# itz-sayak/C-Users-Sayakdutta-Self-Supervised-Arbitrary-Scale-Point-Cloud-Upsampling-via-SNN

Measured on AMD Instinct MI355X. Metric: upsampled query-points/sec (kNN + fn fwd + rotate + fd fwd + displace), 4x scale, M=48 T=4, higher is better.
Workload: dtype f32 (GEMMs as 3 x f16 MFMA with f32 accumulation; outer kNN f64); 1 GPU; synthetic sphere N=5000 (seed 0), B=4096 grid queries per GPU per step, M=48, T=4, fn k=[24,18,12] emb 640, fd k=32 scales [8,16,32,48] emb 768, conditioned-random weights seed 0, in-patch kNN recomputed every batch; cloud_points=5000, neighbours=48, outer_knn=f64 brute force, parallelism=query shards x1

## Files before the change

c-users-sayakdutta-self-supervised-arbitrary-scale-point-cloud-upsampling-via-snn_amd/_lib.py:

```python
import ctypes
import os
from ctypes import POINTER, c_char_p, c_double, c_float, c_int, c_int32, c_int64, c_void_p

_HERE = os.path.dirname(os.path.abspath(__file__))
LIB_PATH = os.environ.get("SAPCU_LIB_PATH") or os.path.join(_HERE, "csrc", "libsapcu_hip.so")
EXACT_LIB_PATH = os.path.join(_HERE, "csrc", "libsapcu_hip_exact.so")

FN_TAPS = ("stem", "block1", "block2", "block3", "pooled", "enc", "logits")
FD_TAPS = ("fused0", "spikes", "knn", "pooled", "enc", "x0")
KIND_FN, KIND_FD = 0, 1
ABI_VERSION = 2


class SapcuLibraryError(RuntimeError):
    """The HIP library is absent or unloadable (never silently replaced by a CPU path)."""


class SapcuError(RuntimeError):
    """A C entry point returned a non-zero status: args = (code, text)."""


_SIGNATURES = {
    "sapcu_abi_version": (c_int, []),
    "sapcu_last_error": (c_char_p, []),
# ... 129 lines not shown
    "sapcu_plan_stats_f64": (c_int, [c_void_p, c_int64, c_void_p, c_int64, c_void_p, c_void_p, c_int, c_double, c_void_p, c_void_p,
                                     c_void_p, c_int64, c_void_p]),
}
SINKHORN_EXPORTS = tuple(_SINKHORN_SIGNATURES)

_RAY_SIGNATURES = {
    "sapcu_ray_mesh_workspace_bytes": (c_int64, [c_int64, c_int64, c_int64]),
    "sapcu_ray_mesh_f64": (c_int, [c_void_p, c_int64, c_void_p, c_int64, c_void_p, c_void_p, c_void_p, c_int64, c_double, c_void_p, c_void_p,
                                   c_void_p, c_void_p, c_int64, POINTER(c_int64), c_void_p]),
    "sapcu_ray_fd_samples_workspace_bytes": (c_int64, [c_int64, c_int64, c_int64]),
    "sapcu_ray_fd_samples_f64": (c_int, [c_void_p, c_int64, c_void_p, c_int64, c_void_p, c_void_p, c_void_p, c_void_p, c_int64, c_double] +
                                 [c_void_p] * 4 + [c_void_p, c_int64, POINTER(c_int64), c_void_p]),
}
RAY_EXPORTS = tuple(_RAY_SIGNATURES)

_NORMALS_SIGNATURES = {
    "sapcu_pca_normals_f64": (c_int, [c_void_p, c_int64, c_void_p, c_int64, c_int, POINTER(c_double), c_void_p, c_void_p, c_void_p, c_void_p]),
    "sapcu_normal_angles_f64": (c_int, [c_void_p, c_void_p, c_int64, c_int, c_double, c_void_p, c_void_p, c_void_p]),
}
NORMALS_EXPORTS = tuple(_NORMALS_SIGNATURES)

_INTERNAL_SIGNATURES = {
    "sapcu_internal_fold_affine_host": (c_int, [c_void_p, c_void_p, c_void_p, c_void_p, c_int, c_int, c_void_p, c_void_p]),
    "sapcu_internal_point_mesh_tuned": (c_int, [c_void_p, c_int64, c_void_p, c_int64, c_void_p, c_int64, c_double, c_double, c_int, c_int, c_void_p,
                                                c_void_p, c_void_p, c_void_p, c_int64, POINTER(c_int64), c_void_p]),
    "sapcu_internal_sinkhorn_split": (c_int, [c_int64, c_int64, POINTER(c_int64)]),
    "sapcu_internal_softmin_split_f64": (c_int, [c_void_p, c_int64, c_void_p, c_int64, c_void_p, c_int, c_double, c_int, c_void_p, c_void_p,
                                                 c_int64, c_void_p]),
    "sapcu_internal_ray_mesh_tuned": (c_int, [c_void_p, c_int64, c_void_p, c_int64, c_void_p, c_void_p, c_void_p, c_int64, c_double, c_double,
                                              c_int, c_double, c_int, c_void_p, c_void_p, c_void_p, c_void_p, c_int64, POINTER(c_int64),
                                              c_void_p]),
}
_lib = None


def load(path=None):
    global _lib
    if _lib is not None and path is None:
        return _lib
    p = path or LIB_PATH
    if not os.path.exists(p):
        raise SapcuLibraryError(
            "HIP library not built: %s is missing. Run `make -C %s` (needs hipcc, gfx950). "
            "There is no CPU fallback." % (p, os.path.dirname(p)))
    try:
        lib = ctypes.CDLL(p)
# ... 34 lines not shown
```

c-users-sayakdutta-self-supervised-arbitrary-scale-point-cloud-upsampling-via-snn_amd/csrc/model.hip:

```cpp
#include <stdarg.h>
#include <stdlib.h>

#include <new>
#include <vector>

#include "common.h"
#include "ops.h"

namespace sapcu {

static thread_local char g_err[512] = "";

void set_error(const char* fmt, ...) {
    va_list ap;
    va_start(ap, fmt);
    vsnprintf(g_err, sizeof(g_err), fmt, ap);
    va_end(ap);
}

enum FnSlot {
    FN_STEM_W = 0, FN_STEM_B, FN_STEM_LIF,
    FN_BLK0 = 3,
    FN_FINAL_W = FN_BLK0 + 63, FN_FINAL_B, FN_FINAL_LIF,
    FN_FCOUT_W, FN_FCOUT_B,
    FN_MLP0_W, FN_MLP0_B, FN_MLP1_W, FN_MLP1_B, FN_MLP2_W, FN_MLP2_B,
    FN_HEAD_W, FN_HEAD_B, FN_LN_W, FN_LN_B,
// ... 35 lines not shown
struct sapcu_model {
    int kind = 0;
    int kv[3] = {0, 0, 0};
    int k = 0, nscale = 0;
    int ks[8] = {0, 0, 0, 0, 0, 0, 0, 0};
    int32_t* ks_dev = nullptr;
    int* gate_dev = nullptr;
    bool sf16 = true;
    void* w16_hi = nullptr;
    void* w16_lo = nullptr;
    void* chain_w = nullptr;
    int* ovf_dev = nullptr;
    int emb = 0, T = 0, heads = 0;
    int64_t chunk = 0;
    int64_t ws_budget = 0;
    bool opt_bt = true;
    bool opt_chain = true;
    bool opt_chain_wide = false;
    bool opt_chain_fill = true;
    bool opt_chain_trim = true;
    bool opt_shortk = true;
    bool opt_fn_maxfuse = true;
    bool opt_fn_fold_out = true;
    bool opt_fd_maxfuse = true;
    bool opt_fd_split = true;
    bool opt_fd_fused = true;
    bool opt_fd_x0 = true;
    void* fde_w = nullptr;
    int64_t fde_off[5] = {0, 0, 0, 0, 0};
    float* fde_nprm = nullptr;
    float* blob = nullptr;
    int64_t blob_floats = 0;
    int64_t fold_w[3] = {0, 0, 0}, fold_b[3] = {0, 0, 0};
    std::vector<int64_t> dir;
    const float* p(int slot) const { return blob + dir[slot]; }
};

namespace sapcu {

static inline int64_t imax(int64_t a, int64_t b) { return a > b ? a : b; }
static inline int imin(int a, int b) { return a < b ? a : b; }

static bool split_rows_gemm_on_big_tile(const GemmArgs& g, bool allow_bt) { return allow_bt && gemm_sf16_bt_ok(g); }

int launch_gemm_split_rows(const GemmArgs& g, hipStream_t st, bool allow_bt) {
    if (split_rows_gemm_on_big_tile(g, allow_bt)) return launch_gemm_sf16_bt(g, st);
    return launch_gemm_sf16_ring(g, st);
}

static void fold_affine_f64(const float* w1, const float* b1, const float* w2, const float* b2, int d, int n, float* w_fold,
                            float* b_fold) {
    std::vector<double> acc((size_t)d);
    for (int i = 0; i < n; ++i) {
        for (int k = 0; k < d; ++k) acc[k] = 0.0;
        double bs = 0.0;
        for (int j = 0; j < d; ++j) {
            const double a = (double)w2[(int64_t)i * d + j];
            const float* row = w1 + (int64_t)j * d;
            for (int k = 0; k < d; ++k) acc[k] += a * (double)row[k];
            bs += a * (double)b1[j];
        }
        for (int k = 0; k < d; ++k) w_fold[(int64_t)i * d + k] = (float)acc[k];
        b_fold[i] = (float)(bs + (double)b2[i]);
    }
}

static bool env_is(const char* name, const char* value) {
    const char* e = getenv(name);
    return e && strcmp(e, value) == 0;
}

static void read_env_switches(sapcu_model* m) {
    m->sf16 = !env_is("SAPCU_GEMM", "f32");
    m->opt_bt = !env_is("SAPCU_BT", "0");
    m->opt_chain = !env_is("SAPCU_CHAIN", "0");
    m->opt_chain_wide = env_is("SAPCU_CHAIN", "wide");
    m->opt_chain_fill = !env_is("SAPCU_CHAIN_FILL", "0");
    m->opt_chain_trim = !env_is("SAPCU_CHAIN_TRIM", "0");
    m->opt_shortk = !env_is("SAPCU_SHORTK", "0");
    m->opt_fn_maxfuse = !env_is("SAPCU_FN_MAXFUSE", "0");
    m->opt_fn_fold_out = !env_is("SAPCU_FN_FOLD_OUT", "0");
    m->opt_fd_maxfuse = !env_is("SAPCU_FD_MAXFUSE", "0");
    m->opt_fd_split = !env_is("SAPCU_FD_SPLIT", "0");
    m->opt_fd_fused = !env_is("SAPCU_FD_FUSED", "0");
    m->opt_fd_x0 = !env_is("SAPCU_FD_X0", "0");
    const char* ce = getenv("SAPCU_CHUNK");
    m->chunk = ce ? atoll(ce) : 0;
    if (m->chunk < 0) m->chunk = 0;
    const char* be = getenv("SAPCU_WS_BUDGET_MB");
    m->ws_budget = (be ? atoll(be) : 20480) * (int64_t)(1 << 20);
    if (m->ws_budget < (int64_t)(64 << 20)) m->ws_budget = (int64_t)(64 << 20);
}

static void free_model(sapcu_model* m) {
    void* const owned[] = {m->w16_hi, m->w16_lo, m->chain_w, m->ovf_dev, m->blob, m->ks_dev, m->gate_dev, m->fde_w, m->fde_nprm};
    for (void* p : owned)
        if (p) (void)hipFree(p);
    delete m;
}

static int run_gemm(const sapcu_model* m, GemmArgs& g, hipStream_t st) {
    const bool have16 = m && m->sf16 && g.w >= m->blob && g.w < m->blob + m->blob_floats;
    if (have16) {
        const int64_t off = g.w - m->blob;
        g.w16_hi = (const _Float16*)m->w16_hi + off;
        g.w16_lo = (const _Float16*)m->w16_lo + off;
        g.ovf = m->ovf_dev;
        if (g.a_split) return launch_gemm_split_rows(g, st, m->opt_bt);
        if (m->opt_shortk && gemm_shortk_ok(g)) return launch_gemm_shortk(g, st);
        if (g.max_out) {
            set_error("run_gemm: a direct max output needs the short-K kernel");
            return SAPCU_ERR_ARG;
        }
        if (g.k % 64 == 0) return launch_gemm_sf16(g, st);
    }
    if (g.a_split || g.c_split || g.c2_split) {
        set_error("run_gemm: split-row operands need the split-f16 kernels");
        return SAPCU_ERR_ARG;
// ... 237 lines not shown
                SAPCU_CHECK_HIP(hipMemcpy2DAsync((char*)taps[SAPCU_FN_TAP_BLOCK1 + l] + s * mp * 64 * 4, 64 * 4,
                                                 out, 192 * 4, 64 * 4, (size_t)P, hipMemcpyDeviceToDevice, st));
            }
            fin = out;
            ldin = 192;
        }
        if (m->sf16 && m->opt_fn_maxfuse) {
            GemmArgs g;
            memset(&g, 0, sizeof(g));
            g.a = W.cat; g.r = P; g.k = 192; g.lda = 192; g.w = m->p(FN_FINAL_W); g.n = m->emb; g.bias = m->p(FN_FINAL_B);
            g.ldc = m->emb; g.epi = EPI_LIF_MAX; g.lif = m->p(FN_FINAL_LIF); g.lif_T = m->T;
            g.max_keys = reinterpret_cast<unsigned*>(W.B1); g.max_m = mp;
            const bool direct = m->opt_shortk && mp == 48;
            if (direct) g.max_out = W.pooled;
            else SAPCU_CHECK_HIP(hipMemsetAsync(g.max_keys, 0, (size_t)cb * m->emb * 4, st));
            SAPCU_TRY(run_gemm(m, g, st));
            if (!direct) SAPCU_TRY(launch_decode_max_keys(g.max_keys, cb * m->emb, W.pooled, st));
        } else {
            SAPCU_TRY(gemm(m, W.cat, P, 192, 192, m->p(FN_FINAL_W), m->emb, m->p(FN_FINAL_B), W.B1, m->emb, EPI_LIF, st,
                           m->p(FN_FINAL_LIF), m->T));
            SAPCU_TRY(launch_rowgroup_max(W.B1, cb, mp, m->emb, W.pooled, st));
        }
        SAPCU_TRY(tap_copy(taps, SAPCU_FN_TAP_POOLED, s * m->emb * 4, W.pooled, cb * m->emb * 4, st));
        SAPCU_TRY(gemm(m, W.pooled, cb, m->emb, m->emb, m->p(FN_FCOUT_W), 2048, m->p(FN_FCOUT_B), W.enc, 2048, EPI_BIAS, st));
        SAPCU_TRY(tap_copy(taps, SAPCU_FN_TAP_ENC, s * 2048 * 4, W.enc, cb * 2048 * 4, st));
        SAPCU_TRY(gemm(m, W.enc, cb, 2048, 2048, m->p(FN_MLP0_W), 1024, m->p(FN_MLP0_B), W.h1, 1024, EPI_GELU, st));
        SAPCU_TRY(gemm(m, W.h1, cb, 1024, 1024, m->p(FN_MLP1_W), 512, m->p(FN_MLP1_B), W.h2, 512, EPI_GELU, st));
        SAPCU_TRY(gemm(m, W.h2, cb, 512, 512, m->p(FN_MLP2_W), 256, m->p(FN_MLP2_B), W.h3, 256, EPI_GELU, st));
        SAPCU_TRY(launch_fn_tail(W.h3, cb, 256, m->p(FN_HEAD_W), m->p(FN_HEAD_B), m->p(FN_LN_W), m->p(FN_LN_B), W.logits,
                                 normals + s * 3, st));
        SAPCU_TRY(tap_copy(taps, SAPCU_FN_TAP_LOGITS, s * 3 * 4, W.logits, cb * 3 * 4, st));
    }
    return SAPCU_OK;
}

struct FdPlan {
    int64_t cb;
    int kmax0, kk;
    bool fused;
    bool x0path;
    bool maxfuse;
    int64_t agg_rows(int mp) const { return maxfuse ? 1 : mp; }
};

static bool fd_encoder_fused(const sapcu_model* m, int mp) {
    return m->sf16 && m->opt_fd_fused && m->fde_w && m->fde_nprm && fd_encoder_ok(mp, m->nscale, m->emb, m->T);
}

static bool fd_x0_path(const sapcu_model* m, int mp) {
// ... 173 lines not shown
    ma.pooled = W.POOLED; ma.tap_spikes = c.tap(SAPCU_FD_TAP_SPIKES); ma.gate = m->gate_dev;
    return launch_fd_msc(ma, st);
}

static int fd_msc_from_slabs(const sapcu_model* m, const FdPlan& pl, const FdWs& W, const FdChunk& c, bool split_spikes, hipStream_t st) {
    const int T = m->T, emb = m->emb;
    const int64_t P = c.P();
    if (c.tap(SAPCU_FD_TAP_SPIKES)) {
        for (int t = 0; t < T; ++t)
            SAPCU_CHECK_HIP(hipMemcpyAsync(c.tap(SAPCU_FD_TAP_SPIKES) + ((int64_t)t * c.b + c.s) * c.mp * 960,
                                           W.SPK + (int64_t)t * P * 960, P * 960 * 4, hipMemcpyDeviceToDevice, st));
    }
    if (pl.maxfuse) {
        GemmArgs mg = fd_msc_gemm_args(m, W, c);
        SAPCU_CHECK_HIP(hipMemsetAsync(mg.max_keys, 0, (size_t)T * c.cb * emb * 4, st));
        mg.a_split = split_spikes ? 1 : 0;
        SAPCU_TRY(run_gemm(m, mg, st));
        return launch_decode_max_keys(mg.max_keys, (int64_t)T * c.cb * emb, W.POOLED, st);
    }
    SAPCU_TRY(gemm(m, W.SPK, (int64_t)T * P, 960, 960, m->p(FD_MSC_W), emb, m->p(FD_MSC_B), W.AGG, emb, EPI_LRELU, st));
    return launch_rowgroup_max(W.AGG, (int64_t)T * c.cb, c.mp, emb, W.POOLED, st);
}

static int fd_temporal_decoder(const sapcu_model* m, const FdWs& W, const FdChunk& c, float* dist, hipStream_t st) {
    const int T = m->T, emb = m->emb;
    const int64_t cb = c.cb, s = c.s;
    if (c.tap(SAPCU_FD_TAP_POOLED)) {
        for (int t = 0; t < T; ++t)
            SAPCU_CHECK_HIP(hipMemcpyAsync(c.tap(SAPCU_FD_TAP_POOLED) + ((int64_t)t * c.b + s) * emb, W.POOLED + (int64_t)t * cb * emb,
                                           cb * emb * 4, hipMemcpyDeviceToDevice, st));
    }
    SAPCU_TRY(launch_fd_temporal(W.POOLED, T, cb, emb, m->p(FD_TI_W), m->p(FD_SNNFC), W.ENC, st));
    SAPCU_TRY(tap_copy(c.taps, SAPCU_FD_TAP_ENC, s * emb * 4, W.ENC, cb * emb * 4, st));
    SAPCU_TRY(gemm(m, W.ENC, cb, emb, emb, m->p(FD_FCIN_W), 256, m->p(FD_FCIN_B), W.D1, 256, EPI_GELU, st));
    SAPCU_TRY(gemm(m, W.D1, cb, 256, 256, m->p(FD_R0_FC0_W), 128, m->p(FD_R0_FC0_B), W.D2a, 128, EPI_GELU, st));
    SAPCU_TRY(gemm(m, W.D1, cb, 256, 256, m->p(FD_R0_PROJ_W), 128, m->p(FD_R0_PROJ_B), W.D2b, 128, EPI_BIAS, st));
    SAPCU_TRY(gemm(m, W.D2a, cb, 128, 128, m->p(FD_R0_FC4_W), 128, m->p(FD_R0_FC4_B), W.D2c, 128, EPI_RESID_GELU, st, nullptr, 0, W.D2b,
                   128));
    SAPCU_TRY(gemm(m, W.D2c, cb, 128, 128, m->p(FD_R1_FC0_W), 64, m->p(FD_R1_FC0_B), W.D3a, 64, EPI_GELU, st));
    SAPCU_TRY(gemm(m, W.D2c, cb, 128, 128, m->p(FD_R1_PROJ_W), 64, m->p(FD_R1_PROJ_B), W.D3b, 64, EPI_BIAS, st));
    SAPCU_TRY(gemm(m, W.D3a, cb, 64, 64, m->p(FD_R1_FC4_W), 64, m->p(FD_R1_FC4_B), W.D3c, 64, EPI_RESID_GELU, st, nullptr, 0, W.D3b, 64));
    SAPCU_TRY(gemm(m, W.D3c, cb, 64, 64, m->p(FD_QKV_W), 192, m->p(FD_QKV_B), W.QKV, 192, EPI_BIAS, st));
    return launch_fd_tail(W.D3c, W.QKV, cb, m->heads, m->p(FD_WO_T), m->p(FD_BO), m->p(FD_LN_W), m->p(FD_LN_B), m->p(FD_WH_T),
                          m->p(FD_BH), m->p(FD_WD), m->p(FD_BD), W.ATT, dist + s, st);
}

static int fd_forward(const sapcu_model* m, const float* patch, int64_t b, int mp, const int32_t* knn_force,
                      float* dist, void* ws, int64_t ws_bytes, void* const* taps, hipStream_t st) {
    const FdPlan pl = fd_plan(m, b, mp);
    const FdWs W = fd_ws_layout(ws_align256(ws), m, pl, mp);
    if (ws_bytes < (int64_t)W.bytes + 256) {
        set_error("fd_forward: workspace %lld B < required %lld B", (long long)ws_bytes, (long long)W.bytes + 256);
        return SAPCU_ERR_WORKSPACE;
// ... 296 lines not shown
            if (m->dir[i] < 0 || m->dir[i] >= blob_floats || (m->dir[i] & 3)) {
                set_error("model_create: slot %d offset %lld out of range / unaligned", i, (long long)m->dir[i]);
                rc = SAPCU_ERR_ARG;
                break;
            }
    }
    auto hip_ok = [&](hipError_t e, const char* what) {
        if (e != hipSuccess && rc == SAPCU_OK) {
            set_error("model_create: %s failed: %s", what, hipGetErrorString(e));
            rc = SAPCU_ERR_HIP;
        }
    };
    if (rc == SAPCU_OK) {
        int64_t total = blob_floats;
        if (kind == SAPCU_KIND_FN && m->opt_fn_fold_out) {
            total = (total + 63) & ~(int64_t)63;
            for (int l = 0; l < 3; ++l) {
                m->fold_w[l] = total;
                total += (int64_t)64 * (128 << l);
                m->fold_b[l] = total;
                total += 64;
            }
        }
        m->blob_floats = total;
        hip_ok(hipMalloc((void**)&m->blob, (size_t)total * 4), "hipMalloc(blob)");
        if (rc == SAPCU_OK) hip_ok(hipMemcpy(m->blob, blob, (size_t)blob_floats * 4, hipMemcpyDeviceToDevice), "copy blob");
        if (rc == SAPCU_OK && total > blob_floats)
            hip_ok(hipMemset(m->blob + blob_floats, 0, (size_t)(total - blob_floats) * 4), "memset folded parameters");
        for (int l = 0; l < 3 && rc == SAPCU_OK && total > blob_floats; ++l) {
            const int d = 128 << l, sb = FN_BLK0 + l * B_SLOTS;
            const int64_t need[4] = {(int64_t)d * d, d, (int64_t)64 * d, 64};
            static const int slot[4] = {B_OUT_W, B_OUT_B, B_FC2_W, B_FC2_B};
            std::vector<float> h[4], wf((size_t)64 * d), bf(64);
            for (int q = 0; q < 4 && rc == SAPCU_OK; ++q) {
                if (m->dir[sb + slot[q]] + need[q] > blob_floats) {
                    set_error("model_create(fn): slot %d runs past the end of the blob", sb + slot[q]);
                    rc = SAPCU_ERR_ARG;
                    break;
                }
                h[q].resize((size_t)need[q]);
                hip_ok(hipMemcpy(h[q].data(), m->p(sb + slot[q]), (size_t)need[q] * 4, hipMemcpyDeviceToHost), "read out_proj / fc2");
            }
            if (rc != SAPCU_OK) break;
            fold_affine_f64(h[0].data(), h[1].data(), h[2].data(), h[3].data(), d, 64, wf.data(), bf.data());
            hip_ok(hipMemcpy(m->blob + m->fold_w[l], wf.data(), wf.size() * 4, hipMemcpyHostToDevice), "copy folded weights");
            if (rc == SAPCU_OK) hip_ok(hipMemcpy(m->blob + m->fold_b[l], bf.data(), bf.size() * 4, hipMemcpyHostToDevice), "copy folded bias");
        }
        if (rc == SAPCU_OK) hip_ok(hipMalloc((void**)&m->ovf_dev, 2 * sizeof(int)), "hipMalloc(ovf)");
        if (rc == SAPCU_OK) hip_ok(hipMemset(m->ovf_dev, 0, 2 * sizeof(int)), "memset ovf");
        if (rc == SAPCU_OK && m->sf16) {
            hip_ok(hipMalloc(&m->w16_hi, (size_t)total * 2), "hipMalloc(w16_hi)");
            if (rc == SAPCU_OK) hip_ok(hipMalloc(&m->w16_lo, (size_t)total * 2), "hipMalloc(w16_lo)");
            if (rc == SAPCU_OK) {
                int wovf = 0;
                if (launch_split_weights(m->blob, total, m->w16_hi, m->w16_lo, m->ovf_dev + 1, nullptr) != SAPCU_OK)
                    rc = SAPCU_ERR_HIP;
                if (rc == SAPCU_OK) hip_ok(hipMemcpy(&wovf, m->ovf_dev + 1, sizeof(int), hipMemcpyDeviceToHost), "read ovf");
                if (rc == SAPCU_OK && wovf != 0) m->sf16 = false;
            }
            if (rc == SAPCU_OK && m->sf16 && kind == SAPCU_KIND_FN) {
                hip_ok(hipMalloc(&m->chain_w, (size_t)chain_w_off(3, 0) * 2), "hipMalloc(chain_w)");
                for (int l = 0; l < 3 && rc == SAPCU_OK; ++l) {
                    const int d = 128 << l;
                    static const int slots[3] = {B_DELTA2_W, B_GAMMA_W, B_GAMMA2_W};
                    for (int q = 0; q < 3 && rc == SAPCU_OK; ++q) {
                        const int64_t wo = m->dir[FN_BLK0 + l * B_SLOTS + slots[q]];
                        if (launch_pack_chain_weights((const _Float16*)m->w16_hi + wo, (const _Float16*)m->w16_lo + wo, d,
                                                      (_Float16*)m->chain_w + chain_w_off(l, q), nullptr) != SAPCU_OK)
                            rc = SAPCU_ERR_HIP;
// ... 9 lines not shown
            if (rc == SAPCU_OK) hip_ok(hipMemset(m->gate_dev, 0, sizeof(int)), "memset gate");
            if (rc == SAPCU_OK && m->sf16 && m->emb >= 96) {
                const int first = m->nscale <= 4 ? 0 : 4;
                const int mats[5][3] = {{FD_FUSE_W, 64, 64 * m->nscale}, {FD_EDGE1_W, 256, 64}, {FD_EDGE2_W, 512, 128},
                                        {FD_EDGE3_W, 1024, 256}, {FD_MSC_W, m->emb, 960}};
                int64_t halves = 0;
                for (int i = 0; i < 5; ++i) {
                    m->fde_off[i] = halves;
                    if (i >= first) halves += (int64_t)2 * mats[i][1] * mats[i][2];
                }
                hip_ok(hipMalloc(&m->fde_w, (size_t)halves * 2), "hipMalloc(fde_w)");
                if (rc == SAPCU_OK) hip_ok(hipMalloc((void**)&m->fde_nprm, 960 * 8 * sizeof(float)), "hipMalloc(fde_nprm)");
                for (int i = first; i < 5 && rc == SAPCU_OK; ++i) {
                    const int64_t wo = m->dir[mats[i][0]];
                    if (launch_pack_frag_weights((const _Float16*)m->w16_hi + wo, (const _Float16*)m->w16_lo + wo, mats[i][1], mats[i][2],
                                                 (_Float16*)m->fde_w + m->fde_off[i], nullptr) != SAPCU_OK)
                        rc = SAPCU_ERR_HIP;
                }
                static const int nslot[4] = {FD_SNN0, FD_SNN1, FD_SNN2, FD_SNN3}, nch[4] = {64, 128, 256, 512}, noff[4] = {0, 64, 192, 448};
                for (int i = 0; i < 4 && rc == SAPCU_OK; ++i)
                    if (launch_pack_fd_neuron(m->p(nslot[i]), nch[i], i < 2 ? 1 : 0, noff[i], m->fde_nprm, nullptr) != SAPCU_OK) rc = SAPCU_ERR_HIP;
                if (rc == SAPCU_OK) hip_ok(hipDeviceSynchronize(), "pack fd encoder operands");
            }
        }
    }
    if (rc != SAPCU_OK) {
        free_model(m);
        return rc;
    }
    *out = m;
    return SAPCU_OK;
}

int sapcu_internal_fold_affine_host(const float* w_out, const float* b_out, const float* w_fc2, const float* b_fc2, int d, int n,
                                    float* w_fold_out, float* b_fold_out) {
    SAPCU_CHECK_ARG(w_out && b_out && w_fc2 && b_fc2 && w_fold_out && b_fold_out && d >= 1 && n >= 1, "fold_affine: bad argument");
    fold_affine_f64(w_out, b_out, w_fc2, b_fc2, d, n, w_fold_out, b_fold_out);
    return SAPCU_OK;
}

int sapcu_model_destroy(sapcu_model_t m) {
    if (!m) return SAPCU_OK;
    free_model(m);
    return SAPCU_OK;
}

int64_t sapcu_workspace_bytes(sapcu_model_t m, int64_t b, int m_pts) {
    if (!m || b < 0 || m_pts < 1 || m_pts > 128) {
        set_error("workspace_bytes: bad argument");
        return SAPCU_ERR_ARG;
    }
    const size_t bytes = m->kind == SAPCU_KIND_FN ? fn_ws_layout(nullptr, m, fn_plan(m, b, m_pts), m_pts).bytes
                                                  : fd_ws_layout(nullptr, m, fd_plan(m, b, m_pts), m_pts).bytes;
    return (int64_t)bytes + 256;
}

int sapcu_model_gate_violations(sapcu_model_t m, int* count_host) {
    SAPCU_CHECK_ARG(m && count_host, "gate_violations: null pointer");
    *count_host = 0;
    if (m->gate_dev) SAPCU_CHECK_HIP(hipMemcpy(count_host, m->gate_dev, sizeof(int), hipMemcpyDeviceToHost));
// ... 44 lines not shown
```

c-users-sayakdutta-self-supervised-arbitrary-scale-point-cloud-upsampling-via-snn_amd/csrc/ops.h:

```cpp
#pragma once
#include "common.h"

namespace sapcu {

int launch_patch_knn_strided(const float* feat, int64_t b, int64_t pstride, int m, int c, int ld, int k,
                             int32_t* idx, hipStream_t st);
int launch_patch_knn_multi(const float* feat, int64_t b, int64_t pstride, int m, int c, int ld, int ntab,
                           const int* ks, int32_t* const* idx, hipStream_t st);
int launch_patch_knn(const float* feat, int64_t b, int m, int c, int ld, int k, int32_t* idx, hipStream_t st);
int launch_neuron_selfloop(const float* x, int64_t rows, int ch, int T, const float* md, const float* ta,
                           const float* rd, const float* tb, const float* dT, const float* rh, float* so, float* mo,
                           float* to, float* ro, hipStream_t st);
int launch_neuron_drive(const float* x, int64_t rows, int ch, int T, const float* md, const float* ta, const float* rd, const float* tb,
                        const float* dT, const float* rh, int pairv, float* so, float* mo, float* to, float* ro, int* gate, hipStream_t st);
int launch_fn_stem(const float* patch, int64_t rows, const float* w, const float* bias, const float* lif, int T,
                   float* out, hipStream_t st);
int launch_fn_pe1(const float* patch, const int32_t* idx, int64_t rows, int m, int kk, int d, const float* w,
                  const float* bias, const float* lif, int T, float* out, int split, hipStream_t st);
struct ChainArgs {
    int64_t P;
    int m;
    const int2* tab;
    const float4* pd;
    const float* qkv;
// ... 70 lines not shown
    int64_t b;
    int64_t b_total, s0;
    int m, T, emb;
    const _Float16* msc_wp;
    const float* msc_b;
    const float* nprm;
    float* pooled;
    float* tap_spikes;
    int* gate;
};
bool fd_msc_ok(int m, int emb, int T);
int launch_fd_msc(const FdMscArgs& a, hipStream_t st);
bool fd_encoder_ok(int m, int nscale, int emb, int T);
int launch_fd_encoder(const FdEncArgs& a, hipStream_t st);
int launch_pack_frag_weights(const void* w16_hi, const void* w16_lo, int n, int k, void* out, hipStream_t st);
int launch_pack_fd_neuron(const float* raw, int C, int eif, int coff, float* out, hipStream_t st);
int launch_fd_pre(const float* in, int ldi, const int32_t* idx, int kk, int m, const float* shift, int64_t pts, int C, float* out,
                  int ldo, int coff, hipStream_t st);
int launch_fd_temporal(const float* pooled, int T, int64_t b, int emb, const float* tw, const float* lif, float* out,
                       hipStream_t st);
int launch_fd_tail(const float* x, const float* qkv, int64_t b, int heads, const float* wo_t, const float* bo,
                   const float* lnw, const float* lnb, const float* wh_t, const float* bh, const float* wd,
                   const float* bd, float* attn_out, float* dist, hipStream_t st);
int64_t train_column_sums_bytes(int64_t rows, int ch);
int train_column_sums(const float* a, int64_t rows, int ch, void* ws, double** sums_out, hipStream_t st);

}
```

Baseline: 133,400 query-points/s.

## Fuse FD head MLP chain into one kernel and fold FN encoder affine

Adds a single fused kernel for the FD head. It runs temporal pooling, the LIF neuron, eight small split-f16 MFMA layers with GELU and residuals, attention, layernorm and the distance head on 16-row tiles held in LDS, replacing a sequence of separate GEMM and tail launches. In the FN path, the fc_out and mlp0 linear layers are folded on the host in f64 into one emb×1024 GEMM, which removes the 2048-wide intermediate. The host fold is multithreaded to cut model-creation time. The risks are low occupancy from 16-row tiles with large LDS, and small numeric drift from the folded weights.

New measurement: 133,900 query-points/s, median of 6. No clear change (+0.4%).

```diff
diff --git a/c-users-sayakdutta-self-supervised-arbitrary-scale-point-cloud-upsampling-via-snn_amd/_lib.py b/c-users-sayakdutta-self-supervised-arbitrary-scale-point-cloud-upsampling-via-snn_amd/_lib.py
--- a/c-users-sayakdutta-self-supervised-arbitrary-scale-point-cloud-upsampling-via-snn_amd/_lib.py
+++ b/c-users-sayakdutta-self-supervised-arbitrary-scale-point-cloud-upsampling-via-snn_amd/_lib.py
@@ -175,6 +175,7 @@
 
 _INTERNAL_SIGNATURES = {
     "sapcu_internal_fold_affine_host": (c_int, [c_void_p, c_void_p, c_void_p, c_void_p, c_int, c_int, c_void_p, c_void_p]),
+    "sapcu_internal_fold_affine_rect_host": (c_int, [c_void_p, c_void_p, c_void_p, c_void_p, c_int, c_int, c_int, c_void_p, c_void_p]),
     "sapcu_internal_point_mesh_tuned": (c_int, [c_void_p, c_int64, c_void_p, c_int64, c_void_p, c_int64, c_double, c_double, c_int, c_int, c_void_p,
                                                 c_void_p, c_void_p, c_void_p, c_int64, POINTER(c_int64), c_void_p]),
     "sapcu_internal_sinkhorn_split": (c_int, [c_int64, c_int64, POINTER(c_int64)]),
diff --git a/c-users-sayakdutta-self-supervised-arbitrary-scale-point-cloud-upsampling-via-snn_amd/csrc/heads.hip b/c-users-sayakdutta-self-supervised-arbitrary-scale-point-cloud-upsampling-via-snn_amd/csrc/heads.hip
--- /dev/null
+++ b/c-users-sayakdutta-self-supervised-arbitrary-scale-point-cloud-upsampling-via-snn_amd/csrc/heads.hip
@@ -0,0 +1,203 @@
+#include "common.h"
+#include "gemm_epi.h"
+#include "ops.h"
+
+namespace sapcu {
+typedef _Float16 half8 __attribute__((ext_vector_type(8)));
+
+constexpr int HD_RT = 16;
+constexpr int HD_NT = 256;
+constexpr int HD_KSTEP = 2 * HD_RT * 64;
+constexpr int HD_P1_BYTES = (256 / 32) * HD_KSTEP;
+constexpr int HD_TAIL_FLOATS = HD_RT * 64 + HD_RT * 192 + 4 * 64 + 64;
+
+__host__ __device__ inline int fd_head_p0_bytes(int emb) { return ((emb > 128 ? emb : 128) / 32) * HD_KSTEP; }
+static int fd_head_lds_bytes(int emb) { return fd_head_p0_bytes(emb) + HD_P1_BYTES + HD_TAIL_FLOATS * 4; }
+
+__device__ __forceinline__ unsigned hd_panel_off(int row, int k) {
+    return (unsigned)((k >> 5) * HD_KSTEP + row * 64 + ((((k >> 3) & 3) ^ ((row >> 2) & 3)) << 4) + (k & 7) * 2);
+}
+__device__ __forceinline__ void hd_put(unsigned char* X, int row, int k, float v, bool count, bool& bad) {
+    unsigned char* p = X + hd_panel_off(row, k);
+    v = settle(v);
+    const _Float16 hi = (_Float16)v;
+    *reinterpret_cast<_Float16*>(p) = hi;
+    *reinterpret_cast<_Float16*>(p + HD_RT * 64) = (_Float16)(v - (float)hi);
+    bad = bad || (count && fabsf(v) > 65504.0f);
+}
+
+template <int NCS>
+__device__ __forceinline__ void hd_gemm(const unsigned char* X, const half8* __restrict__ wp, int nk32, int cs0, int lane, f32x4 (&acc)[NCS]) {
+    const int c16 = lane & 15, g = lane >> 4;
+    const unsigned char* xa = X + c16 * 64 + ((g ^ ((c16 >> 2) & 3)) * 16);
+    half8 wh[NCS], wl[NCS];
+#pragma unroll
+    for (int j = 0; j < NCS; ++j) {
+        acc[j] = f32x4{0.f, 0.f, 0.f, 0.f};
+        wh[j] = wp[((int64_t)(cs0 + j) * nk32 * 2) * 64 + lane];
+        wl[j] = wp[((int64_t)(cs0 + j) * nk32 * 2 + 1) * 64 + lane];
+    }
+#pragma unroll 1
+    for (int s = 0; s < nk32; ++s) {
+        const int sn = s + 1 < nk32 ? s + 1 : s;
+        half8 nh[NCS], nl[NCS];
+#pragma unroll
+        for (int j = 0; j < NCS; ++j) {
+            nh[j] = wp[(((int64_t)(cs0 + j) * nk32 + sn) * 2) * 64 + lane];
+            nl[j] = wp[(((int64_t)(cs0 + j) * nk32 + sn) * 2 + 1) * 64 + lane];
+        }
+        const half8 ah = *reinterpret_cast<const half8*>(xa + s * HD_KSTEP);
+        const half8 al = *reinterpret_cast<const half8*>(xa + s * HD_KSTEP + HD_RT * 64);
+#pragma unroll
+        for (int j = 0; j < NCS; ++j) acc[j] = __builtin_amdgcn_mfma_f32_16x16x32_f16(al, wh[j], acc[j], 0, 0, 0);
+#pragma unroll
+        for (int j = 0; j < NCS; ++j) acc[j] = __builtin_amdgcn_mfma_f32_16x16x32_f16(ah, wl[j], acc[j], 0, 0, 0);
+#pragma unroll
+        for (int j = 0; j < NCS; ++j) acc[j] = __builtin_amdgcn_mfma_f32_16x16x32_f16(ah, wh[j], acc[j], 0, 0, 0);
+#pragma unroll
+        for (int j = 0; j < NCS; ++j) {
+            wh[j] = nh[j];
+            wl[j] = nl[j];
+        }
+    }
+}
+
+template <int NCS, typename Out>
+__device__ __forceinline__ void hd_layer(const unsigned char* X, int k, const _Float16* __restrict__ wp, const float* __restrict__ bias,
+                                         int wave, int lane, Out out) {
+    f32x4 acc[NCS];
+    const int cs0 = wave * NCS;
+    hd_gemm<NCS>(X, reinterpret_cast<const half8*>(wp), k / 32, cs0, lane, acc);
+#pragma unroll
+    for (int j = 0; j < NCS; ++j) {
+        const int col = 16 * (cs0 + j) + (lane & 15);
+        const float bv = bias[col];
+#pragma unroll
+        for (int e = 0; e < 4; ++e) out(j, e, 4 * (lane >> 4) + e, col, __fadd_rn(__fmul_rn(acc[j][e], 0.0625f), bv));
+    }
+}
+
+__device__ __forceinline__ float hd_wave_sum(float v) {
+#pragma unroll
+    for (int o = 32; o >= 1; o >>= 1) v += __shfl_xor(v, o);
+    return v;
+}
+
+__global__ __launch_bounds__(HD_NT) void fd_head_kernel(const FdHeadArgs a) {
+    extern __shared__ __attribute__((aligned(16))) unsigned char hd_smem[];
+    unsigned char* P0 = hd_smem;
+    unsigned char* P1 = hd_smem + fd_head_p0_bytes(a.emb);
+    float* XS = reinterpret_cast<float*>(P1 + HD_P1_BYTES);
+    float* QS = XS + HD_RT * 64;
+    float* SH = QS + HD_RT * 192;
+    float* TW = SH + 4 * 64;
+    const int tid = threadIdx.x, lane = tid & 63, wave = tid >> 6;
+    const int64_t row0 = (int64_t)blockIdx.x * HD_RT;
+    const int emb = a.emb, T = a.T;
+    bool bad = false;
+
+    if (tid < T) {
+        float mx = a.tw[0];
+        for (int i = 1; i < T; ++i) mx = fmaxf(mx, a.tw[i]);
+        float den = 0.f;
+        for (int i = 0; i < T; ++i) den = __fadd_rn(den, expf(__fsub_rn(a.tw[i], mx)));
+        TW[tid] = __fdiv_rn(expf(__fsub_rn(a.tw[tid], mx)), den);
+    }
+    __syncthreads();
+    for (int f = tid; f < emb; f += HD_NT) {
+        const NeuronP p = load_lif(a.lif, emb, f);
+        for (int r = 0; r < HD_RT; ++r) {
+            const int64_t row = row0 + r;
+            const bool valid = row < a.b;
+            float acc = 0.f;
+            for (int i = 0; i < T; ++i) acc = __fmaf_rn(TW[i], valid ? a.pooled[((int64_t)i * a.b + row) * emb + f] : 0.f, acc);
+            NeuronS s = neuron_init(p);
+            hd_put(P0, r, f, neuron_step<false>(acc, s, p), valid, bad);
+        }
+    }
+    __syncthreads();
+
+    const bool rows_ok[4] = {row0 + 4 * (lane >> 4) < a.b, row0 + 4 * (lane >> 4) + 1 < a.b, row0 + 4 * (lane >> 4) + 2 < a.b,
+                             row0 + 4 * (lane >> 4) + 3 < a.b};
+    hd_layer<4>(P0, emb, a.wp[0], a.bias[0], wave, lane, [&](int, int e, int r, int col, float v) { hd_put(P1, r, col, gelu_erf(v), rows_ok[e], bad); });
+    __syncthreads();
+    float res0[2][4];
+    hd_layer<2>(P1, 256, a.wp[1], a.bias[1], wave, lane, [&](int, int e, int r, int col, float v) { hd_put(P0, r, col, gelu_erf(v), rows_ok[e], bad); });
+    hd_layer<2>(P1, 256, a.wp[2], a.bias[2], wave, lane, [&](int j, int e, int, int, float v) { res0[j][e] = v; });
+    __syncthreads();
+    hd_layer<2>(P0, 128, a.wp[3], a.bias[3], wave, lane,
+                [&](int j, int e, int r, int col, float v) { hd_put(P1, r, col, gelu_erf(__fadd_rn(v, res0[j][e])), rows_ok[e], bad); });
+    __syncthreads();
+    float res1[1][4];
+    hd_layer<1>(P1, 128, a.wp[4], a.bias[4], wave, lane, [&](int, int e, int r, int col, float v) { hd_put(P0, r, col, gelu_erf(v), rows_ok[e], bad); });
+    hd_layer<1>(P1, 128, a.wp[5], a.bias[5], wave, lane, [&](int j, int e, int, int, float v) { res1[j][e] = v; });
+    __syncthreads();
+    hd_layer<1>(P0, 64, a.wp[6], a.bias[6], wave, lane, [&](int j, int e, int r, int col, float v) {
+        const float y = gelu_erf(__fadd_rn(v, res1[j][e]));
+        hd_put(P1, r, col, y, rows_ok[e], bad);
+        XS[r * 64 + col] = y;
+    });
+    __syncthreads();
+    hd_layer<3>(P1, 64, a.wp[7], a.bias[7], wave, lane, [&](int, int, int r, int col, float v) { QS[r * 192 + col] = v; });
+    __syncthreads();
+    if (__any(bad) && lane == 0 && a.ovf) atomicAdd(a.ovf, 1);
+
+    const int hd = 64 / a.heads;
+    float* sh = SH + wave * 64;
+    for (int i = 0; i < HD_RT / 4; ++i) {
+        const int r = wave * (HD_RT / 4) + i;
+        const int64_t row = row0 + r;
+        if (row >= a.b) break;
+        const float q = QS[r * 192 + lane], k = QS[r * 192 + 64 + lane], v = QS[r * 192 + 128 + lane];
+        float dot = q * k;
+        for (int o = 1; o < hd; o <<= 1) dot += __shfl_xor(dot, o);
+        const float logit = dot * (1.0f / sqrtf((float)hd));
+        float mx = logit;
+        for (int o = hd; o < 64; o <<= 1) mx = fmaxf(mx, __shfl_xor(mx, o));
+        const float e = expf(logit - mx);
+        float den = e;
+        for (int o = hd; o < 64; o <<= 1) den += __shfl_xor(den, o);
+        const float o_c = (e / den) * v;
+        __builtin_amdgcn_wave_barrier();
+        sh[lane] = o_c;
+        __builtin_amdgcn_wave_barrier();
+        float acc = a.bo[lane];
+        for (int c = 0; c < 64; ++c) acc = fmaf(sh[c], a.wo_t[c * 64 + lane], acc);
+        const float y = acc + XS[r * 64 + lane];
+        const float mean = hd_wave_sum(y) / 64.0f;
+        const float dc = y - mean;
+        const float var = hd_wave_sum(dc * dc) / 64.0f;
+        const float z = dc * (1.0f / sqrtf(var + 1e-5f)) * a.lnw[lane] + a.lnb[lane];
+        __builtin_amdgcn_wave_barrier();
+        sh[lane] = z;
+        __builtin_amdgcn_wave_barrier();
+        float hsum = 0.f;
+        if (lane < 32) {
+            hsum = a.bh[lane];
+            for (int c = 0; c < 64; ++c) hsum = fmaf(sh[c], a.wh_t[c * 32 + lane], hsum);
+            hsum = gelu_erf(hsum) * a.wd[lane];
+        }
+        const float tot = hd_wave_sum(hsum) + a.bd[0];
+        if (lane == 0) {
+            const float bx = 5.0f * tot;
+            a.dist[row] = bx > 20.0f ? tot : log1pf(expf(bx)) / 5.0f;
+        }
+    }
+}
+
+bool fd_head_ok(int emb, int heads, int T) {
+    return emb >= 64 && emb % 64 == 0 && emb <= 1024 && heads >= 1 && heads <= 64 && (heads & (heads - 1)) == 0 && T >= 1 && T <= 64;
+}
+
+int launch_fd_head(const FdHeadArgs& a, hipStream_t st) {
+    if (a.b == 0) return SAPCU_OK;
+    SAPCU_CHECK_ARG(fd_head_ok(a.emb, a.heads, a.T), "fd_head: unsupported shape (emb=%d heads=%d T=%d)", a.emb, a.heads, a.T);
+    static DeviceOnce lds_once;
+    const int lds = fd_head_lds_bytes(1024);
+    SAPCU_SET_MAX_LDS(lds_once, fd_head_kernel, lds);
+    hipLaunchKernelGGL(fd_head_kernel, dim3((unsigned)((a.b + HD_RT - 1) / HD_RT)), dim3(HD_NT), fd_head_lds_bytes(a.emb), st, a);
+    SAPCU_CHECK_LAUNCH();
+    return SAPCU_OK;
+}
+
+}
diff --git a/c-users-sayakdutta-self-supervised-arbitrary-scale-point-cloud-upsampling-via-snn_amd/csrc/model.hip b/c-users-sayakdutta-self-supervised-arbitrary-scale-point-cloud-upsampling-via-snn_amd/csrc/model.hip
--- a/c-users-sayakdutta-self-supervised-arbitrary-scale-point-cloud-upsampling-via-snn_amd/csrc/model.hip
+++ b/c-users-sayakdutta-self-supervised-arbitrary-scale-point-cloud-upsampling-via-snn_amd/csrc/model.hip
@@ -2,6 +2,7 @@
 #include <stdlib.h>
 
 #include <new>
+#include <thread>
 #include <vector>
 
 #include "common.h"
@@ -83,16 +84,21 @@
     bool opt_shortk = true;
     bool opt_fn_maxfuse = true;
     bool opt_fn_fold_out = true;
+    bool opt_fn_fold_enc = true;
     bool opt_fd_maxfuse = true;
     bool opt_fd_split = true;
     bool opt_fd_fused = true;
+    bool opt_head_fuse = true;
     bool opt_fd_x0 = true;
     void* fde_w = nullptr;
     int64_t fde_off[5] = {0, 0, 0, 0, 0};
     float* fde_nprm = nullptr;
+    void* head_w = nullptr;
+    int64_t head_off[8] = {0, 0, 0, 0, 0, 0, 0, 0};
     float* blob = nullptr;
     int64_t blob_floats = 0;
     int64_t fold_w[3] = {0, 0, 0}, fold_b[3] = {0, 0, 0};
+    int64_t fold_enc_w = 0, fold_enc_b = 0;
     std::vector<int64_t> dir;
     const float* p(int slot) const { return blob + dir[slot]; }
 };
@@ -109,21 +115,36 @@
     return launch_gemm_sf16_ring(g, st);
 }
 
-static void fold_affine_f64(const float* w1, const float* b1, const float* w2, const float* b2, int d, int n, float* w_fold,
+static void fold_affine_rows_f64(const float* w1, const float* b1, const float* w2, const float* b2, int dk, int dm, int i0, int i1,
+                                 float* w_fold, float* b_fold) {
+    std::vector<double> acc((size_t)dk);
+    for (int i = i0; i < i1; ++i) {
+        for (int k = 0; k < dk; ++k) acc[k] = 0.0;
+        double bs = 0.0;
+        for (int j = 0; j < dm; ++j) {
+            const double a = (double)w2[(int64_t)i * dm + j];
+            const float* row = w1 + (int64_t)j * dk;
+            for (int k = 0; k < dk; ++k) acc[k] += a * (double)row[k];
+            bs += a * (double)b1[j];
+        }
+        for (int k = 0; k < dk; ++k) w_fold[(int64_t)i * dk + k] = (float)acc[k];
+        b_fold[i] = (float)(bs + (double)b2[i]);
+    }
+}
+
+static void fold_affine_f64(const float* w1, const float* b1, const float* w2, const float* b2, int dk, int dm, int n, float* w_fold,
                             float* b_fold) {
-    std::vector<double> acc((size_t)d);
-    for (int i = 0; i < n; ++i) {
-        for (int k = 0; k < d; ++k) acc[k] = 0.0;
-        double bs = 0.0;
-        for (int j = 0; j < d; ++j) {
-            const double a = (double)w2[(int64_t)i * d + j];
-            const float* row = w1 + (int64_t)j * d;
-            for (int k = 0; k < d; ++k) acc[k] += a * (double)row[k];
-            bs += a * (double)b1[j];
-        }
-        for (int k = 0; k < d; ++k) w_fold[(int64_t)i * d + k] = (float)acc[k];
-        b_fold[i] = (float)(bs + (double)b2[i]);
-    }
+    const int64_t products = (int64_t)n * dm * dk;
+    int nt = products >= ((int64_t)1 << 27) ? 8 : 1;
+    if (nt > n) nt = n;
+    std::vector<std::thread> pool;
+    const int per = (n + nt - 1) / nt;
+    for (int t = 1; t < nt; ++t) {
+        const int i0 = t * per, i1 = imin(n, i0 + per);
+        if (i0 < i1) pool.emplace_back(fold_affine_rows_f64, w1, b1, w2, b2, dk, dm, i0, i1, w_fold, b_fold);
+    }
+    fold_affine_rows_f64(w1, b1, w2, b2, dk, dm, 0, imin(n, per), w_fold, b_fold);
+    for (std::thread& th : pool) th.join();
 }
 
 static bool env_is(const char* name, const char* value) {
@@ -141,10 +162,12 @@
     m->opt_shortk = !env_is("SAPCU_SHORTK", "0");
     m->opt_fn_maxfuse = !env_is("SAPCU_FN_MAXFUSE", "0");
     m->opt_fn_fold_out = !env_is("SAPCU_FN_FOLD_OUT", "0");
+    m->opt_fn_fold_enc = !env_is("SAPCU_FN_FOLD_ENC", "0");
     m->opt_fd_maxfuse = !env_is("SAPCU_FD_MAXFUSE", "0");
     m->opt_fd_split = !env_is("SAPCU_FD_SPLIT", "0");
     m->opt_fd_fused = !env_is("SAPCU_FD_FUSED", "0");
     m->opt_fd_x0 = !env_is("SAPCU_FD_X0", "0");
+    m->opt_head_fuse = !env_is("SAPCU_HEAD_FUSE", "0");
     const char* ce = getenv("SAPCU_CHUNK");
     m->chunk = ce ? atoll(ce) : 0;
     if (m->chunk < 0) m->chunk = 0;
@@ -154,7 +177,7 @@
 }
 
 static void free_model(sapcu_model* m) {
-    void* const owned[] = {m->w16_hi, m->w16_lo, m->chain_w, m->ovf_dev, m->blob, m->ks_dev, m->gate_dev, m->fde_w, m->fde_nprm};
+    void* const owned[] = {m->w16_hi, m->w16_lo, m->chain_w, m->ovf_dev, m->blob, m->ks_dev, m->gate_dev, m->fde_w, m->fde_nprm, m->head_w};
     for (void* p : owned)
         if (p) (void)hipFree(p);
     delete m;
@@ -438,9 +461,16 @@
             SAPCU_TRY(launch_rowgroup_max(W.B1, cb, mp, m->emb, W.pooled, st));
         }
         SAPCU_TRY(tap_copy(taps, SAPCU_FN_TAP_POOLED, s * m->emb * 4, W.pooled, cb * m->emb * 4, st));
-        SAPCU_TRY(gemm(m, W.pooled, cb, m->emb, m->emb, m->p(FN_FCOUT_W), 2048, m->p(FN_FCOUT_B), W.enc, 2048, EPI_BIAS, st));
-        SAPCU_TRY(tap_copy(taps, SAPCU_FN_TAP_ENC, s * 2048 * 4, W.enc, cb * 2048 * 4, st));
-        SAPCU_TRY(gemm(m, W.enc, cb, 2048, 2048, m->p(FN_MLP0_W), 1024, m->p(FN_MLP0_B), W.h1, 1024, EPI_GELU, st));
+        const bool fold_enc = m->fold_enc_w > 0;
+        if (!fold_enc || (taps && taps[SAPCU_FN_TAP_ENC])) {
+            SAPCU_TRY(gemm(m, W.pooled, cb, m->emb, m->emb, m->p(FN_FCOUT_W), 2048, m->p(FN_FCOUT_B), W.enc, 2048, EPI_BIAS, st));
+            SAPCU_TRY(tap_copy(taps, SAPCU_FN_TAP_ENC, s * 2048 * 4, W.enc, cb * 2048 * 4, st));
+        }
+        if (fold_enc)
+            SAPCU_TRY(gemm(m, W.pooled, cb, m->emb, m->emb, m->blob + m->fold_enc_w, 1024, m->blob + m->fold_enc_b, W.h1, 1024, EPI_GELU,
+                           st));
+        else
+            SAPCU_TRY(gemm(m, W.enc, cb, 2048, 2048, m->p(FN_MLP0_W), 1024, m->p(FN_MLP0_B), W.h1, 1024, EPI_GELU, st));
         SAPCU_TRY(gemm(m, W.h1, cb, 1024, 1024, m->p(FN_MLP1_W), 512, m->p(FN_MLP1_B), W.h2, 512, EPI_GELU, st));
         SAPCU_TRY(gemm(m, W.h2, cb, 512, 512, m->p(FN_MLP2_W), 256, m->p(FN_MLP2_B), W.h3, 256, EPI_GELU, st));
         SAPCU_TRY(launch_fn_tail(W.h3, cb, 256, m->p(FN_HEAD_W), m->p(FN_HEAD_B), m->p(FN_LN_W), m->p(FN_LN_B), W.logits,
@@ -660,6 +690,11 @@
     return launch_rowgroup_max(W.AGG, (int64_t)T * c.cb, c.mp, emb, W.POOLED, st);
 }
 
+static const int FD_HEAD_MATS[8][3] = {{FD_FCIN_W, 256, 0},   {FD_R0_FC0_W, 128, 256}, {FD_R0_PROJ_W, 128, 256}, {FD_R0_FC4_W, 128, 128},
+                                       {FD_R1_FC0_W, 64, 128}, {FD_R1_PROJ_W, 64, 128}, {FD_R1_FC4_W, 64, 64},    {FD_QKV_W, 192, 64}};
+
+static bool fd_head_fused(const sapcu_model* m) { return m->sf16 && m->opt_head_fuse && m->head_w; }
+
 static int fd_temporal_decoder(const sapcu_model* m, const FdWs& W, const FdChunk& c, float* dist, hipStream_t st) {
     const int T = m->T, emb = m->emb;
     const int64_t cb = c.cb, s = c.s;
@@ -667,6 +702,20 @@
         for (int t = 0; t < T; ++t)
             SAPCU_CHECK_HIP(hipMemcpyAsync(c.tap(SAPCU_FD_TAP_POOLED) + ((int64_t)t * c.b + s) * emb, W.POOLED + (int64_t)t * cb * emb,
                                            cb * emb * 4, hipMemcpyDeviceToDevice, st));
+    }
+    if (fd_head_fused(m) && !c.tap(SAPCU_FD_TAP_ENC)) {
+        FdHeadArgs ha;
+        memset(&ha, 0, sizeof(ha));
+        ha.pooled = W.POOLED; ha.b = cb; ha.T = T; ha.emb = emb; ha.heads = m->heads;
+        ha.tw = m->p(FD_TI_W); ha.lif = m->p(FD_SNNFC);
+        for (int i = 0; i < 8; ++i) {
+            ha.wp[i] = (const _Float16*)m->head_w + m->head_off[i];
+            ha.bias[i] = m->p(FD_HEAD_MATS[i][0] + 1);
+        }
+        ha.wo_t = m->p(FD_WO_T); ha.bo = m->p(FD_BO); ha.lnw = m->p(FD_LN_W); ha.lnb = m->p(FD_LN_B);
+        ha.wh_t = m->p(FD_WH_T); ha.bh = m->p(FD_BH); ha.wd = m->p(FD_WD); ha.bd = m->p(FD_BD);
+        ha.dist = dist + s; ha.ovf = m->ovf_dev;
+        return launch_fd_head(ha, st);
     }
     SAPCU_TRY(launch_fd_temporal(W.POOLED, T, cb, emb, m->p(FD_TI_W), m->p(FD_SNNFC), W.ENC, st));
     SAPCU_TRY(tap_copy(c.taps, SAPCU_FD_TAP_ENC, s * emb * 4, W.ENC, cb * emb * 4, st));
@@ -1009,12 +1058,19 @@
                 total += 64;
             }
         }
+        if (kind == SAPCU_KIND_FN && m->opt_fn_fold_enc) {
+            total = (total + 63) & ~(int64_t)63;
+            m->fold_enc_w = total;
+            total += (int64_t)1024 * m->emb;
+            m->fold_enc_b = total;
+            total += 1024;
+        }
         m->blob_floats = total;
         hip_ok(hipMalloc((void**)&m->blob, (size_t)total * 4), "hipMalloc(blob)");
         if (rc == SAPCU_OK) hip_ok(hipMemcpy(m->blob, blob, (size_t)blob_floats * 4, hipMemcpyDeviceToDevice), "copy blob");
         if (rc == SAPCU_OK && total > blob_floats)
             hip_ok(hipMemset(m->blob + blob_floats, 0, (size_t)(total - blob_floats) * 4), "memset folded parameters");
-        for (int l = 0; l < 3 && rc == SAPCU_OK && total > blob_floats; ++l) {
+        for (int l = 0; l < 3 && rc == SAPCU_OK && m->fold_w[0] > 0; ++l) {
             const int d = 128 << l, sb = FN_BLK0 + l * B_SLOTS;
             const int64_t need[4] = {(int64_t)d * d, d, (int64_t)64 * d, 64};
             static const int slot[4] = {B_OUT_W, B_OUT_B, B_FC2_W, B_FC2_B};
@@ -1029,9 +1085,29 @@
                 hip_ok(hipMemcpy(h[q].data(), m->p(sb + slot[q]), (size_t)need[q] * 4, hipMemcpyDeviceToHost), "read out_proj / fc2");
             }
             if (rc != SAPCU_OK) break;
-            fold_affine_f64(h[0].data(), h[1].data(), h[2].data(), h[3].data(), d, 64, wf.data(), bf.data());
+            fold_affine_f64(h[0].data(), h[1].data(), h[2].data(), h[3].data(), d, d, 64, wf.data(), bf.data());
             hip_ok(hipMemcpy(m->blob + m->fold_w[l], wf.data(), wf.size() * 4, hipMemcpyHostToDevice), "copy folded weights");
             if (rc == SAPCU_OK) hip_ok(hipMemcpy(m->blob + m->fold_b[l], bf.data(), bf.size() * 4, hipMemcpyHostToDevice), "copy folded bias");
+        }
+        if (rc == SAPCU_OK && m->fold_enc_w > 0) {
+            const int emb = m->emb;
+            const int64_t need[4] = {(int64_t)2048 * emb, 2048, (int64_t)1024 * 2048, 1024};
+            static const int slot[4] = {FN_FCOUT_W, FN_FCOUT_B, FN_MLP0_W, FN_MLP0_B};
+            std::vector<float> h[4], wf((size_t)1024 * emb), bf(1024);
+            for (int q = 0; q < 4 && rc == SAPCU_OK; ++q) {
+                if (m->dir[slot[q]] + need[q] > blob_floats) {
+                    set_error("model_create(fn): slot %d runs past the end of the blob", slot[q]);
+                    rc = SAPCU_ERR_ARG;
+                    break;
+                }
+                h[q].resize((size_t)need[q]);
+                hip_ok(hipMemcpy(h[q].data(), m->p(slot[q]), (size_t)need[q] * 4, hipMemcpyDeviceToHost), "read fc_out / mlp0");
+            }
+            if (rc == SAPCU_OK) {
+                fold_affine_f64(h[0].data(), h[1].data(), h[2].data(), h[3].data(), emb, 2048, 1024, wf.data(), bf.data());
+                hip_ok(hipMemcpy(m->blob + m->fold_enc_w, wf.data(), wf.size() * 4, hipMemcpyHostToDevice), "copy folded weights");
+            }
+            if (rc == SAPCU_OK) hip_ok(hipMemcpy(m->blob + m->fold_enc_b, bf.data(), bf.size() * 4, hipMemcpyHostToDevice), "copy folded bias");
         }
         if (rc == SAPCU_OK) hip_ok(hipMalloc((void**)&m->ovf_dev, 2 * sizeof(int)), "hipMalloc(ovf)");
         if (rc == SAPCU_OK) hip_ok(hipMemset(m->ovf_dev, 0, 2 * sizeof(int)), "memset ovf");
@@ -1087,6 +1163,26 @@
                     if (launch_pack_fd_neuron(m->p(nslot[i]), nch[i], i < 2 ? 1 : 0, noff[i], m->fde_nprm, nullptr) != SAPCU_OK) rc = SAPCU_ERR_HIP;
                 if (rc == SAPCU_OK) hip_ok(hipDeviceSynchronize(), "pack fd encoder operands");
             }
+            if (rc == SAPCU_OK && m->sf16 && m->opt_head_fuse && fd_head_ok(m->emb, m->heads, m->T)) {
+                int64_t halves = 0;
+                for (int i = 0; i < 8; ++i) {
+                    m->head_off[i] = halves;
+                    halves += (int64_t)2 * FD_HEAD_MATS[i][1] * (FD_HEAD_MATS[i][2] ? FD_HEAD_MATS[i][2] : m->emb);
+                }
+                hip_ok(hipMalloc(&m->head_w, (size_t)halves * 2), "hipMalloc(head_w)");
+                for (int i = 0; i < 8 && rc == SAPCU_OK; ++i) {
+                    const int n = FD_HEAD_MATS[i][1], k = FD_HEAD_MATS[i][2] ? FD_HEAD_MATS[i][2] : m->emb;
+                    const int64_t wo = m->dir[FD_HEAD_MATS[i][0]];
+                    if (wo + (int64_t)n * k > blob_floats) {
+                        set_error("model_create(fd): slot %d runs past the end of the blob", FD_HEAD_MATS[i][0]);
+                        rc = SAPCU_ERR_ARG;
+                    } else if (launch_pack_frag_weights((const _Float16*)m->w16_hi + wo, (const _Float16*)m->w16_lo + wo, n, k,
+                                                        (_Float16*)m->head_w + m->head_off[i], nullptr) != SAPCU_OK) {
+                        rc = SAPCU_ERR_HIP;
+                    }
+                }
+                if (rc == SAPCU_OK) hip_ok(hipDeviceSynchronize(), "pack fd head operands");
+            }
         }
     }
     if (rc != SAPCU_OK) {
@@ -1100,7 +1196,14 @@
 int sapcu_internal_fold_affine_host(const float* w_out, const float* b_out, const float* w_fc2, const float* b_fc2, int d, int n,
                                     float* w_fold_out, float* b_fold_out) {
     SAPCU_CHECK_ARG(w_out && b_out && w_fc2 && b_fc2 && w_fold_out && b_fold_out && d >= 1 && n >= 1, "fold_affine: bad argument");
-    fold_affine_f64(w_out, b_out, w_fc2, b_fc2, d, n, w_fold_out, b_fold_out);
+    fold_affine_f64(w_out, b_out, w_fc2, b_fc2, d, d, n, w_fold_out, b_fold_out);
+    return SAPCU_OK;
+}
+
+int sapcu_internal_fold_affine_rect_host(const float* w1, const float* b1, const float* w2, const float* b2, int dk, int dm, int n,
+                                         float* w_fold_out, float* b_fold_out) {
+    SAPCU_CHECK_ARG(w1 && b1 && w2 && b2 && w_fold_out && b_fold_out && dk >= 1 && dm >= 1 && n >= 1, "fold_affine_rect: bad argument");
+    fold_affine_f64(w1, b1, w2, b2, dk, dm, n, w_fold_out, b_fold_out);
     return SAPCU_OK;
 }
 
diff --git a/c-users-sayakdutta-self-supervised-arbitrary-scale-point-cloud-upsampling-via-snn_amd/csrc/ops.h b/c-users-sayakdutta-self-supervised-arbitrary-scale-point-cloud-upsampling-via-snn_amd/csrc/ops.h
--- a/c-users-sayakdutta-self-supervised-arbitrary-scale-point-cloud-upsampling-via-snn_amd/csrc/ops.h
+++ b/c-users-sayakdutta-self-supervised-arbitrary-scale-point-cloud-upsampling-via-snn_amd/csrc/ops.h
@@ -116,6 +116,20 @@
 int launch_fd_tail(const float* x, const float* qkv, int64_t b, int heads, const float* wo_t, const float* bo,
                    const float* lnw, const float* lnb, const float* wh_t, const float* bh, const float* wd,
                    const float* bd, float* attn_out, float* dist, hipStream_t st);
+struct FdHeadArgs {
+    const float* pooled;
+    int64_t b;
+    int T, emb, heads;
+    const float* tw;
+    const float* lif;
+    const _Float16* wp[8];
+    const float* bias[8];
+    const float *wo_t, *bo, *lnw, *lnb, *wh_t, *bh, *wd, *bd;
+    float* dist;
+    int* ovf;
+};
+bool fd_head_ok(int emb, int heads, int T);
+int launch_fd_head(const FdHeadArgs& a, hipStream_t st);
 int64_t train_column_sums_bytes(int64_t rows, int ch);
 int train_column_sums(const float* a, int64_t rows, int ch, void* ws, double** sums_out, hipStream_t st);
 
```
